# jasonyaw/CDAE

Hardware: AMD Instinct MI355X
Metric: users/sec (whole node) K=200 ML-10M-shape; Recall@10 parity (higher is better)
Workload: dtype f32

## Files before the change

cdae_amd/csrc/cdae_hip.hip:

```cpp
#include <hip/hip_runtime.h>

#include <cstring>

#include <rocprim/rocprim.hpp>

#include <algorithm>
#include <atomic>
#include <condition_variable>
#include <deque>
#include <mutex>
#include <thread>
#include <chrono>
#include <cmath>
#include <cstdarg>
#include <cstdlib>
#include <cstdio>
#include <cstring>
#include <numeric>
#include <string>
#include <vector>

#include "../../include/cdae_hip.h"
#include "cdae_internal.hpp"
#include "cdae_kernels.hpp"
#include "cdae_full_kernels.hpp"
#include "cdae_recommend_kernels.hpp"
#include "cdae_sort_kernels.hpp"
#include "cdae_mf_kernels.hpp"

#ifdef CDAE_DECODE_TIMING
#define CDAE_TOUCHED_ARG ((uint32_t*)nullptr)
#else
#define CDAE_TOUCHED_ARG h->d_touched
#endif

namespace {

thread_local std::string g_err;

int fail(const char* fmt, ...) {
  char buf[1024];
  va_list ap;
  va_start(ap, fmt);
  vsnprintf(buf, sizeof buf, fmt, ap);
  va_end(ap);
  g_err = buf;
  return 1;
}

#define HIPCHK(expr)                                                                           \
  do {                                                                                         \
    hipError_t e__ = (expr);                                                                   \
    if (e__ != hipSuccess)                                                                     \
      return fail("%s failed: %s (%s:%d)", #expr, hipGetErrorString(e__), __FILE__, __LINE__); \
  } while (0)

#define CHK(expr)            \
  do {                       \
    int rc__ = (expr);       \
    if (rc__) return rc__;   \
  } while (0)

#define DISPATCH_NI(ni, KERNEL, grid, block, shmem, stream, ...)                                  \
  do {                                                                                            \
    switch (ni) {                                                                                 \
      case 1: hipLaunchKernelGGL(KERNEL<1>, grid, block, shmem, stream, __VA_ARGS__); break;      \
      case 2: hipLaunchKernelGGL(KERNEL<2>, grid, block, shmem, stream, __VA_ARGS__); break;      \
      case 4: hipLaunchKernelGGL(KERNEL<4>, grid, block, shmem, stream, __VA_ARGS__); break;      \
      default: hipLaunchKernelGGL(KERNEL<8>, grid, block, shmem, stream, __VA_ARGS__); break;     \
    }                                                                                             \
  } while (0)

constexpr uint32_t MF_SEQ_USERS = 256;
constexpr uint32_t ENCODE_USERS_MAX = 768;
enum Family { F_SAMPLE = 0, F_SORT, F_ENCODE, F_DECODE, F_HIDDEN, F_INPUT, F_COUNT };

struct Span { int family; hipEvent_t a, b; };

}
// ... 1311 lines not shown
  CHK(dev_alloc(&h->d_shared, h->n_shared));
  HIPCHK(hipMemset(h->d_shared, 0, h->n_shared * sizeof(float)));
  const size_t WR = (size_t)h->wu_rows();
  h->cnt[CDAE_P_WU] = h->cnt[CDAE_P_WU_AG] = WR * h->Kp;
  CHK(dev_alloc(&h->d_Wu, WR * h->Kp));
  CHK(dev_alloc(&h->d_Wu_ag, WR * h->Kp));
  HIPCHK(hipMemset(h->d_Wu, 0, std::max<size_t>(WR * h->Kp, 1) * sizeof(float)));
  HIPCHK(hipMemset(h->d_Wu_ag, 0, std::max<size_t>(WR * h->Kp, 1) * sizeof(float)));
  if (h->cfg.linear_function) {
    h->cnt[CDAE_P_UU] = h->cnt[CDAE_P_UU_AG] = WR * h->Kp;
    CHK(dev_alloc(&h->d_Uu, WR * h->Kp));
    CHK(dev_alloc(&h->d_Uu_ag, WR * h->Kp));
  }

  const uint32_t B = (uint32_t)std::min<uint64_t>(h->B, U);
  uint64_t emax = 0;
  for (uint64_t s0 = 0; s0 < U; ++s0) {
    const uint64_t s1 = std::min<uint64_t>(U, s0 + B);
    emax = std::max<uint64_t>(emax, (uint64_t)(row_ptr[s1] - row_ptr[s0]));
  }
  h->ex_per_pos = h->mf == 2 ? 2u * h->hp.num_neg : 1u + h->hp.num_neg;
  h->Ecap = emax * h->ex_per_pos;
  h->h_grow_ptr.clear(); h->h_gunit_ptr.clear();
  if (h->shard_sampled()) {
    const int64_t* grp = h->g_row_ptr_src;
    const uint32_t* gcl = h->g_col_src;
    h->g_row_ptr_src = nullptr; h->g_col_src = nullptr;
    if (grp[0] != 0) return fail("whole-row row_ptr[0] must be 0");
    h->h_grow_ptr.assign(grp, grp + U + 1);
    uint64_t gmax = 0;
    for (uint64_t s0 = 0; s0 < U; ++s0) gmax = std::max<uint64_t>(gmax, (uint64_t)(grp[std::min<uint64_t>(U, s0 + B)] - grp[s0]));
    h->Ecap = gmax * h->ex_per_pos;
    const size_t gnnz = (size_t)grp[U];
    CHK(dev_alloc(&h->d_grow_ptr, U + 1)); CHK(dev_alloc(&h->d_gcol, gnnz));
    HIPCHK(hipMemcpy(h->d_grow_ptr, grp, (U + 1) * sizeof(int64_t), hipMemcpyHostToDevice));
    HIPCHK(hipMemcpy(h->d_gcol, gcl, gnnz * sizeof(uint32_t), hipMemcpyHostToDevice));
    h->h_gunit_ptr.assign(U + 1, 0u);
    for (uint64_t u = 0; u < U; ++u)
      h->h_gunit_ptr[u + 1] = h->h_gunit_ptr[u] + (uint32_t)((grp[u + 1] - grp[u] + h->hp.unit_pos - 1) / h->hp.unit_pos);
    CHK(dev_alloc(&h->d_gunit_ptr, U + 1));
    HIPCHK(hipMemcpy(h->d_gunit_ptr, h->h_gunit_ptr.data(), (U + 1) * sizeof(uint32_t), hipMemcpyHostToDevice));
    std::vector<uint32_t> guser(h->h_gunit_ptr[U]);
    for (uint64_t u = 0; u < U; ++u)
      for (uint32_t g = h->h_gunit_ptr[u]; g < h->h_gunit_ptr[u + 1]; ++g) guser[g] = (uint32_t)u;
    CHK(dev_alloc(&h->d_gunit_user, std::max<size_t>(guser.size(), 1)));
    HIPCHK(hipMemcpy(h->d_gunit_user, guser.data(), guser.size() * sizeof(uint32_t), hipMemcpyHostToDevice));
  }
  h->seq = 0; h->pre_n = 0;
  h->counting_sort = I <= cdae::TILE_SORT_MAX_ITEMS && DEV_ENV("CDAE_SORT_TILE") != nullptr;
  h->bucket_sort = false; h->bucket_ranges = 0; h->cell_units = 0;
  {
    const uint64_t BUCKET_MAX_EXAMPLES = h->cfg.full_output ? 100000 : 600000;
    const uint64_t keys = I + (h->shard_sampled() ? 1u : 0u);
    if (keys <= 65536 && !h->counting_sort && !h->mf_seq && h->Ecap <= BUCKET_MAX_EXAMPLES && h->Ecap > 0 && !DEV_ENV("CDAE_SORT_LIBRARY")) {
      const double b_share = (double)B / (double)U;
      const double draw_items = (double)(h->shard_sampled() ? h->I_global : I);
      const double whole_nnz = h->shard_sampled() ? (double)h->h_grow_ptr[U] : (double)nnz;
      const uint32_t negs = h->mf == 2 ? 2u * h->hp.num_neg - 0u : h->hp.num_neg;
      const double neg_per_item = b_share * whole_nnz * (double)negs / draw_items;
      std::vector<double> wgt(I);
      double total = 0.0;
      for (uint64_t i = 0; i < I; ++i) { wgt[i] = b_share * (double)pop[i] + neg_per_item; total += wgt[i]; }
      const double per_range = std::max(total / 256.0, std::min(2730.0, total / 8.0));
      std::vector<uint32_t> cut{0u};
      double acc = 0.0;
      for (uint64_t i = 0; i < I; ++i) {
        acc += wgt[i];
        if (i + 1 < I && (acc >= per_range || (i + 1) - cut.back() == cdae::BK_ITEMS)) { cut.push_back((uint32_t)(i + 1)); acc = 0.0; }
      }
      cut.push_back((uint32_t)I);
      if (cut.size() - 1 <= cdae::BK_MAX_RANGES) {
        h->bucket_sort = true;
        h->bucket_ranges = (uint32_t)cut.size() - 1;
        CHK(dev_alloc(&h->d_bucket_cut, cut.size()));
        HIPCHK(hipMemcpy(h->d_bucket_cut, cut.data(), cut.size() * sizeof(uint32_t), hipMemcpyHostToDevice));
        if (!h->mf && h->bucket_ranges <= cdae::BKC_MAX_RANGES && h->Ecap < (1ull << (32 - cdae::BKC_ITEM_BITS)) && !DEV_ENV("CDAE_SORT_SCAN")) {
          std::vector<uint16_t> rof(I);
          for (uint32_t r = 0; r + 1 < cut.size(); ++r)
            for (uint32_t i = cut[r]; i < cut[r + 1]; ++i) rof[i] = (uint16_t)r;
          CHK(dev_alloc(&h->d_range_of, (size_t)I));
          HIPCHK(hipMemcpy(h->d_range_of, rof.data(), I * sizeof(uint16_t), hipMemcpyHostToDevice));
        }
      }
    }
  }
  h->h_unit_ptr.assign(U + 1, 0u);
  for (uint64_t u = 0; u < U; ++u)
    h->h_unit_ptr[u + 1] = h->h_unit_ptr[u] + (uint32_t)((row_ptr[u + 1] - row_ptr[u] + h->hp.unit_pos - 1) / h->hp.unit_pos);
  h->unit_cap = 0;
  for (uint64_t s0 = 0; s0 < U; ++s0) {
    const uint64_t s1 = std::min<uint64_t>(U, s0 + B);
    h->unit_cap = std::max(h->unit_cap, h->h_unit_ptr[s1] - h->h_unit_ptr[s0]);
  }
  {
    std::vector<uint32_t> per(U);
    for (uint64_t u = 0; u < U; ++u) per[u] = h->h_unit_ptr[u + 1] - h->h_unit_ptr[u];
    std::partial_sort(per.begin(), per.begin() + B, per.end(), std::greater<uint32_t>());
    uint64_t top = 0;
    for (uint32_t i = 0; i < B; ++i) top += per[i];
    h->unit_cap = (uint32_t)std::max<uint64_t>(h->unit_cap, top);
  }
  if (h->shard_sampled())
    for (uint64_t s0 = 0; s0 < U; ++s0)
      h->unit_cap = std::max(h->unit_cap, h->h_gunit_ptr[std::min<uint64_t>(U, s0 + B)] - h->h_gunit_ptr[s0]);
  CHK(dev_alloc(&h->d_unit_ptr, U + 1));
  HIPCHK(hipMemcpy(h->d_unit_ptr, h->h_unit_ptr.data(), (U + 1) * sizeof(uint32_t), hipMemcpyHostToDevice));
  {
    std::vector<uint32_t> unit_user(h->h_unit_ptr[U]);
    for (uint64_t u = 0; u < U; ++u)
      for (uint32_t g = h->h_unit_ptr[u]; g < h->h_unit_ptr[u + 1]; ++g) unit_user[g] = (uint32_t)u;
    CHK(dev_alloc(&h->d_unit_user, std::max<size_t>(unit_user.size(), 1)));
    HIPCHK(hipMemcpy(h->d_unit_user, unit_user.data(), unit_user.size() * sizeof(uint32_t), hipMemcpyHostToDevice));
  }
  CHK(dev_alloc(&h->d_Hpart, (size_t)h->unit_cap * h->Kp));
  CHK(dev_alloc(&h->d_uptr_tmp, (size_t)B + 1));
  {
    const uint32_t one_unit[2] = {0u, 1u};
    HIPCHK(hipMemcpy(h->d_uptr_tmp, one_unit, sizeof one_unit, hipMemcpyHostToDevice));
  }
  if ((uint64_t)B * h->Kp * sizeof(float) > 0x7FFFFFFFull)
    return fail("batch_users %u x row stride %u floats exceeds the 2 GiB the batch's Z may occupy; lower batch_users", B, h->Kp);
  if (h->Ecap > 0xFFFFFFF0ull) return fail("batch of %u users holds %llu examples (> 2^32); lower batch_users", B, (unsigned long long)h->Ecap);
  for (auto& b : h->ex) {
// ... 1410 lines not shown
```

cdae_amd/csrc/cdae_kernels.hpp:

```cpp
#pragma once
#include <type_traits>

#include <hip/hip_runtime.h>
#include <stdint.h>

#include "../../include/cdae_rng.h"
#include "cdae_exchange_algebra.h"

namespace cdae {

constexpr int WAVE = 64;
constexpr uint32_t SLOT_MASK = 0x0FFFFFFFu;
constexpr uint32_t DUP_PREV_BIT = 1u << 28;
constexpr uint32_t DUP_NEXT_BIT = 1u << 29;
constexpr uint32_t DUP_NONE = 0xFFFFFFFFu;
constexpr uint32_t DUP_STRIPES = 64;
constexpr uint32_t TARGET_BIT = 1u << 30;
constexpr uint32_t INPUT_BIT = 1u << 31;

constexpr uint32_t LATE_MAX = 64;
struct DecodeLate {
  float* Ghot;
  uint32_t* hotdup;
  uint32_t late_rows;
// ... 1393 lines not shown
      if (dup) { const uint32_t k = len + (uint32_t)__popcll(dmask & below); lrow[k] = cur.di[h2] | DUP_ROW; lg[k] = 1.f; }
      if (mine) { const uint32_t k = len + n_d + (uint32_t)__popcll(mask & below); lrow[k] = cur.item[h2]; lg[k] = cur.g[h2]; }
      len += n_d + n_r;
    }
    __builtin_amdgcn_fence(__ATOMIC_RELEASE, "wavefront");
    __builtin_amdgcn_wave_barrier();
    const bool last = c0 + 2 * WAVE >= n_ex;
    while (len - head >= (uint32_t)TRIP) trip((uint32_t)TRIP);
    if (last || len + 4u * WAVE > GCAP) {
      if (len > head) trip(len - head);
      head = 0; len = 0;
      __builtin_amdgcn_wave_barrier();
    }
    cur = nxt;
  }
  if (lo >= hp.K) {
#pragma unroll
    for (int i = 0; i < NI; ++i) acc[i] = 0.f;
  }
  vstore<NI>(ga.HGpart + ((size_t)part * ga.n_units + unit) * hp.Kp + lo, acc);
  trace_end(hp, 5, unit * 8u + part, t0, n_ex);
}

template <int NI>
__global__ void __launch_bounds__(256)
hidden_gather_kernel(HyperParams hp, const int64_t* __restrict__ row_ptr, const uint32_t* __restrict__ uptr,
                     uint32_t n_units, uint64_t u0, uint32_t nb, const uint32_t* __restrict__ ex_item,
                     const float* __restrict__ G, const float* __restrict__ D0,
                     float* __restrict__ HGpart ,
                     uint32_t explicit_examples ,
                     const uint32_t* __restrict__ dup_of_ex, const float* __restrict__ dup_corr,
                     const uint32_t* __restrict__ unit_user,
                     const uint32_t* __restrict__ late_bits = nullptr ,
                     uint32_t late_words = 0) {
  __shared__ uint32_t gl_row[4][GATHER_CAP];
  __shared__ float gl_g[4][GATHER_CAP];
  __shared__ uint32_t lbits[LATE_BITS_WORDS];
  stage_late_bits(lbits, late_bits, late_words);
  const uint32_t part = blockIdx.x & 7u;
  const uint32_t unit = (blockIdx.x >> 3) * (blockDim.x / WAVE) + threadIdx.x / WAVE;
  if (unit >= n_units) return;
  const GatherArgs ga{row_ptr, uptr, n_units, u0, nb, ex_item, G, D0, HGpart, explicit_examples, dup_of_ex, dup_corr, unit_user,
                      late_bits, late_words, nullptr};
  hidden_gather_role<NI, false>(hp, ga, part, unit, gl_row[threadIdx.x / WAVE], gl_g[threadIdx.x / WAVE], late_bits ? lbits : nullptr);
}

struct FusedGeom {
  uint32_t hot_wgs;
  uint32_t decode_wgs;
  const uint32_t* cold_map;
};
constexpr uint32_t FUSED_LDS_WORDS = 4u * 2u * GATHER_CAP + LATE_BITS_WORDS;
static_assert(4u * ROWS16_LDS_WORDS <= FUSED_LDS_WORDS, "row roles' LDS");
static_assert(3u * (FUSED_LDS_WORDS + 8u) * 4u + 90376u <= 160u * 1024u, "three workgroups of this launch + one of bucket_sort_kernel per CU");
#ifndef CDAE_FUSED_WAVES_PER_SIMD
#define CDAE_FUSED_WAVES_PER_SIMD 3
#endif
template <int NV, int NT, int LOSS, bool ADAGRAD>
__global__ void __launch_bounds__(256, CDAE_FUSED_WAVES_PER_SIMD)
decode_gather_kernel(HyperParams hp, uint32_t hot_rows, FusedGeom geo, DecodeLate late, GatherArgs ga, CDAE_DECODE_PARAMS) {
  constexpr int CH = NT == 0 ? NV : NV + 1;
  constexpr int NI = CH <= 1 ? 1 : (CH <= 2 ? 2 : 4);
  __shared__ uint32_t fused_lds[FUSED_LDS_WORDS + 8u];
  const uint32_t wg = blockIdx.x;
  const uint32_t wid = __builtin_amdgcn_readfirstlane(threadIdx.x / WAVE);
  if (wg < geo.hot_wgs) {
    const uint32_t row = wg * 4u + wid;
    if (row < hot_rows && !CDAE_SKIP_ROLE(hp, 4u)) {
      const unsigned long long t0 = trace_begin(hp);
      __builtin_amdgcn_s_setprio(CDAE_HOT_PRIO);
      decode_row64<NI, LOSS, ADAGRAD, false, true>(hp, row, reinterpret_cast<float*>(fused_lds + wid * ROWS16_LDS_WORDS), ROW64_PARK_WORDS, late,
                                                   CDAE_DECODE_PASS);
      __builtin_amdgcn_s_setprio(0);
      trace_end(hp, 3, row, t0, hp.trace ? hw_place() : 0u);
    }
  } else if (wg < geo.decode_wgs) {
    if (CDAE_SKIP_ROLE(hp, 8u)) return;
    uint32_t* const claim = fused_lds + FUSED_LDS_WORDS;
    if (threadIdx.x < 4) claim[threadIdx.x] = 0u;
    __syncthreads();
    const uint32_t simd = (__builtin_amdgcn_s_getreg((1 << 11) | (4 << 6) | 4) ) & 3u;
    if (threadIdx.x % WAVE == 0) atomicCAS(&claim[simd], 0u, 1u + wid);
    __syncthreads();
    const uint32_t cs[4] = {claim[0], claim[1], claim[2], claim[3]};
    int mine = -1;
#pragma unroll
    for (int q = 0; q < 4; ++q) if (cs[q] == 1u + wid) mine = q;
    if (mine < 0) {
      uint32_t before = 0, cnt = 0;
#pragma unroll
      for (int q = 0; q < 4; ++q) if (cs[q] && cs[q] - 1u < wid) ++before;
      const uint32_t j = wid - before;
#pragma unroll
      for (int q = 0; q < 4; ++q) if (!cs[q]) { if (cnt == j) mine = q; ++cnt; }
    }
    const uint32_t g = geo.cold_map[wg * 4u + (uint32_t)mine];
    if (g == 0xFFFFFFFFu) return;
    const unsigned long long t0 = trace_begin(hp);
    decode_rows16<NV, NT, LOSS, ADAGRAD, true>(hp, hot_rows + g * 4u, fused_lds + wid * ROWS16_LDS_WORDS, CDAE_DECODE_PASS);
    trace_end(hp, 4, hot_rows / 4u + g, t0, hp.trace ? hw_place() : 0u);
  } else {
    uint32_t* const lbits = fused_lds + 4u * 2u * GATHER_CAP;
    stage_late_bits(lbits, ga.late_bits, ga.late_words);
    const uint32_t gw = wg - geo.decode_wgs;
    const uint32_t part = gw & 7u, unit = (gw >> 3) * 4u + wid;
    if (unit >= ga.n_units) return;
    hidden_gather_role<NI, true>(hp, ga, part, unit, fused_lds + wid * 2u * GATHER_CAP,
// ... 718 lines not shown
```

cdae_amd/csrc/cdae_sort_kernels.hpp:

```cpp
#pragma once
#include <hip/hip_runtime.h>
#include <stdint.h>

#include "cdae_kernels.hpp"

namespace cdae {

#ifndef CDAE_SEGSORT_THREADS
#define CDAE_SEGSORT_THREADS 256
#endif
constexpr uint32_t SEGSORT_THREADS = CDAE_SEGSORT_THREADS;
#ifndef CDAE_SEGSORT_ITEMS
#define CDAE_SEGSORT_ITEMS 8
#endif
constexpr uint32_t SEGSORT_ITEMS = CDAE_SEGSORT_ITEMS;
#ifndef CDAE_SEGSORT_WINDOW
#define CDAE_SEGSORT_WINDOW 3072
#endif
constexpr uint32_t SEGSORT_WINDOW = CDAE_SEGSORT_WINDOW;

constexpr uint32_t TILE_SORT_MAX_ITEMS = 32768;
#ifndef CDAE_TILE_EX
#define CDAE_TILE_EX 4096
#endif
// ... 143 lines not shown
        const uint64_t v = raw[q];
        uint32_t r[8] = {0, 0, 0, 0, 0, 0, 0, 0};
        uint32_t j = a;
        for (; j + 8 <= b; j += 8) {
#pragma unroll
          for (int t = 0; t < 8; ++t) r[t] += raw[j + t] < v ? 1u : 0u;
        }
        for (; j < b; ++j) r[0] += raw[j] < v ? 1u : 0u;
        rank = ((r[0] + r[1]) + (r[2] + r[3])) + ((r[4] + r[5]) + (r[6] + r[7]));
        srt[a + rank] = v;
      } else {
        const uint64_t v = bucketed_val[p0 + q];
        for (uint32_t j = a; j < b; ++j) rank += bucketed_val[p0 + j] < v ? 1u : 0u;
        sorted_val[p0 + a + rank] = v;
      }
    }
    __syncthreads();
    uint32_t my_dups = 0;
    for (uint32_t q = threadIdx.x; q < n; q += blockDim.x) {
      const uint32_t k = item_of(k0, p0 + q);
      const uint32_t a = item_off[k] - p0, b = item_off[k + 1] - p0;
      uint64_t v = in_lds ? srt[q] : sorted_val[p0 + q];
      const uint32_t slot = (uint32_t)v & SLOT_MASK;
      uint32_t flags = 0;
      if (q > a && ((uint32_t)(in_lds ? srt[q - 1] : sorted_val[p0 + q - 1]) & SLOT_MASK) == slot) flags |= DUP_PREV_BIT;
      if (q + 1 < b && ((uint32_t)(in_lds ? srt[q + 1] : sorted_val[p0 + q + 1]) & SLOT_MASK) == slot) flags |= DUP_NEXT_BIT;
      if (in_lds || flags) sorted_val[p0 + q] = v | flags;
      if (flags & DUP_PREV_BIT) ++my_dups;
    }
    uint32_t off = my_dups ? atomicAdd(&blk_count, my_dups) : 0u;
    __syncthreads();
    if (threadIdx.x == 0) { blk_base = blk_count ? atomicAdd(dup_count + blockIdx.x % stripes, blk_count) : 0u; blk_count = 0u; }
    __syncthreads();
    if (my_dups) {
      off += blk_base;
      const uint32_t stripe_cap = dup_cap / stripes, stripe0 = (blockIdx.x % stripes) * stripe_cap;
      for (uint32_t q = threadIdx.x; q < n; q += blockDim.x) {
        const uint64_t v = sorted_val[p0 + q];
        if (!((uint32_t)v & DUP_PREV_BIT)) continue;
        const uint32_t idx = off < stripe_cap ? stripe0 + off : DUP_NONE;
        ++off;
        dup_of_pos[p0 + q] = idx;
        dup_of_ex[(uint32_t)(v >> 32)] = idx;
      }
    }
    __syncthreads();
    k0 = k1;
  }
}

constexpr uint32_t BK_THREADS = 512;
constexpr uint32_t BK_WINDOW = 4096;
constexpr uint32_t BK_ITEMS = 2048;
constexpr uint32_t BK_WAVE_LIST = BK_WINDOW / (BK_THREADS / 64);
constexpr uint32_t BK_SPIN_CAP = 1u << 21;
constexpr uint32_t BK_MAX_RANGES = 1024;
constexpr uint32_t BK_CELL_UNITS_MAX = 16384;
constexpr size_t BK_LDS_BYTES = (size_t)BK_WINDOW * 8 * 2 + (size_t)BK_WINDOW * 2 + (size_t)(BK_ITEMS + 1) * 4 * 2 + 64 * 4;
static_assert(BK_ITEMS <= 4 * BK_THREADS && BK_ITEMS <= (1u << BKC_ITEM_BITS), "bk_block_scan takes 4 counters per thread; a cell entry holds the item in BKC_ITEM_BITS bits");

__device__ __forceinline__ void bk_block_scan(uint32_t* v, uint32_t n, uint32_t* wave_tot) {
  const uint32_t t = threadIdx.x, lane = t % WAVE, wid = t / WAVE;
  uint32_t c[4], sum = 0;
#pragma unroll
  for (uint32_t j = 0; j < 4; ++j) { c[j] = 4u * t + j < n ? v[4u * t + j] : 0u; sum += c[j]; }
  uint32_t incl = sum;
#pragma unroll
  for (int off = 1; off < WAVE; off <<= 1) {
    const uint32_t o = __shfl_up(incl, off, WAVE);
    if ((int)lane >= off) incl += o;
  }
  if (lane == WAVE - 1) wave_tot[wid] = incl;
  __syncthreads();
  uint32_t before = 0;
  for (uint32_t w = 0; w < wid; ++w) before += wave_tot[w];
  uint32_t run = before + incl - sum;
#pragma unroll
  for (uint32_t j = 0; j < 4; ++j) { if (4u * t + j < n) v[4u * t + j] = run; run += c[j]; }
  if (t == BK_THREADS - 1) v[n] = run;
  __syncthreads();
}

constexpr uint32_t BK_UNROLL = 4;
template <typename F>
__device__ __forceinline__ void bk_scan_keys(const uint16_t* __restrict__ keys, uint32_t n_ex, F&& f) {
  const uint32_t n8 = n_ex & ~7u;
  constexpr uint32_t ROUND = BK_THREADS * 8u * BK_UNROLL;
  uint4 q[BK_UNROLL], nx[BK_UNROLL];
  auto request = [&](uint4 (&dst)[BK_UNROLL], uint32_t r0) {
#pragma unroll
    for (uint32_t u = 0; u < BK_UNROLL; ++u) {
      const uint32_t e0 = r0 + (u * BK_THREADS + threadIdx.x) * 8u;
      dst[u] = e0 < n8 ? *reinterpret_cast<const uint4*>(keys + e0) : make_uint4(0xFFFFFFFFu, 0xFFFFFFFFu, 0xFFFFFFFFu, 0xFFFFFFFFu);
    }
  };
  request(q, 0u);
  for (uint32_t r0 = 0; r0 < n8; r0 += ROUND) {
    const bool more = r0 + ROUND < n8;
    if (more) request(nx, r0 + ROUND);
#pragma unroll
    for (uint32_t u = 0; u < BK_UNROLL; ++u) {
      const uint32_t e0 = r0 + (u * BK_THREADS + threadIdx.x) * 8u;
      if (r0 + u * BK_THREADS * 8u >= n8) break;
      const bool valid = e0 < n8;
      const uint32_t w[4] = {q[u].x, q[u].y, q[u].z, q[u].w};
#pragma unroll
      for (uint32_t j = 0; j < 4; ++j) { f(e0 + 2u * j, w[j] & 0xFFFFu, valid); f(e0 + 2u * j + 1u, w[j] >> 16, valid); }
    }
    if (more) {
#pragma unroll
      for (uint32_t u = 0; u < BK_UNROLL; ++u) q[u] = nx[u];
    }
  }
  if (n_ex != n8 && threadIdx.x < WAVE) {
    const bool valid = threadIdx.x < n_ex - n8;
    f(n8 + threadIdx.x, valid ? (uint32_t)keys[n8 + threadIdx.x] : 0u, valid);
  }
}

__global__ void __launch_bounds__(BK_THREADS)
bucket_sort_kernel(const uint16_t* __restrict__ keys, const uint64_t* __restrict__ ex_val, uint32_t n_ex,
                   const uint32_t* __restrict__ range_cut , uint32_t* __restrict__ wg_state ,
                   const uint32_t* __restrict__ cells , uint32_t cell_units,
                   const uint32_t* __restrict__ cell_flag , uint32_t cell_tag,
                   uint32_t* __restrict__ seg_begin, uint32_t* __restrict__ seg_end, const uint32_t* __restrict__ rank_of,
                   uint32_t* __restrict__ segr_begin, uint32_t* __restrict__ segr_end, uint64_t* __restrict__ sorted_val,
                   uint64_t* __restrict__ scratch_val ,
                   uint32_t* __restrict__ dup_count, uint32_t dup_cap, uint32_t* __restrict__ dup_of_pos,
                   uint32_t* __restrict__ dup_of_ex , uint32_t stripes,
                   uint32_t* __restrict__ err ) {
#ifdef CDAE_PREP_SETPRIO
  __builtin_amdgcn_s_setprio(CDAE_PREP_SETPRIO);
#endif
  extern __shared__ __attribute__((aligned(16))) unsigned char bk_lds[];
  uint64_t* raw = reinterpret_cast<uint64_t*>(bk_lds);
  uint64_t* srt = raw + BK_WINDOW;
  uint32_t* off = reinterpret_cast<uint32_t*>(srt + BK_WINDOW);
  uint32_t* cur = off + BK_ITEMS + 1;
  uint32_t* misc = cur + BK_ITEMS + 1;
  uint16_t* raw_item = reinterpret_cast<uint16_t*>(misc + 64);
  const uint32_t t = threadIdx.x, w = blockIdx.x, lane = t % WAVE;
  const uint32_t lo = range_cut[w], n_it = range_cut[w + 1] - lo;
  for (uint32_t i = t; i <= n_it; i += BK_THREADS) off[i] = 0u;
  if (t == 0) { misc[16] = 0u; misc[17] = 0u; misc[19] = 0u; }
  __syncthreads();

  bool listed = false;
  bool scanned = false;
  if (cells && cell_units <= BK_CELL_UNITS_MAX && *cell_flag != cell_tag) {
    uint16_t* wcnt = reinterpret_cast<uint16_t*>(raw);
    uint32_t* lst = reinterpret_cast<uint32_t*>(srt);
    uint16_t* tk = reinterpret_cast<uint16_t*>(lst + BK_WINDOW);
    const uint32_t* mine = cells + (size_t)w * cell_units * BKC_SLOTS;
    const uint32_t per = (cell_units + BK_THREADS - 1) / BK_THREADS, u0 = min(cell_units, t * per), u1 = min(cell_units, u0 + per);
    uint32_t sum = 0;
    for (uint32_t u = u0; u < u1; ++u) { const uint32_t c = mine[(size_t)u * BKC_SLOTS]; wcnt[u] = (uint16_t)c; sum += c; }
    uint32_t incl = sum;
#pragma unroll
    for (int o = 1; o < WAVE; o <<= 1) {
      const uint32_t v = __shfl_up(incl, o, WAVE);
      if ((int)lane >= o) incl += v;
    }
    if (lane == WAVE - 1) misc[t / WAVE] = incl;
    __syncthreads();
    uint32_t pos = incl - sum, total = 0;
    for (uint32_t v = 0; v < BK_THREADS / WAVE; ++v) { if (v < t / WAVE) pos += misc[v]; total += misc[v]; }
    __syncthreads();
    if (total <= BK_WINDOW) {
      for (uint32_t u = u0; u < u1; ++u) {
        const uint32_t c = wcnt[u];
        for (uint32_t j = 0; j < c; ++j) lst[pos + j] = mine[(size_t)u * BKC_SLOTS + 1u + j];
        pos += c;
      }
      __syncthreads();
      for (uint32_t i = t; i < total; i += BK_THREADS) tk[i] = (uint16_t)atomicAdd(&off[lst[i] & BKC_ITEM_MASK], 1u);
      __syncthreads();
      bk_block_scan(off, n_it, misc);
      for (uint32_t i = t; i < total; i += BK_THREADS) {
        const uint32_t ent = lst[i], d = ent & BKC_ITEM_MASK, p = off[d] + tk[i];
        raw[p] = ex_val[ent >> BKC_ITEM_BITS];
        raw_item[p] = (uint16_t)d;
      }
      listed = true; scanned = true;
    } else {
      for (uint32_t i = t; i <= n_it; i += BK_THREADS) off[i] = 0u;
      __syncthreads();
    }
  }

  uint64_t* const wave_list = srt + (t / WAVE) * BK_WAVE_LIST;
  uint32_t wave_n = 0;
  if (!scanned) {
    bk_scan_keys(keys, n_ex, [&](uint32_t e, uint32_t k, bool valid) {
      const uint32_t d = k - lo;
      const bool mine = valid && d < n_it;
      const uint64_t m = __ballot(mine);
      if (m == 0ull) return;
      if (mine) {
        const uint32_t ticket = atomicAdd(&off[d], 1u);
        const uint32_t slot = wave_n + __builtin_amdgcn_mbcnt_hi((uint32_t)(m >> 32), __builtin_amdgcn_mbcnt_lo((uint32_t)m, 0u));
        if (slot < BK_WAVE_LIST) wave_list[slot] = ((uint64_t)e << 32) | (uint64_t)(d << 16) | (uint64_t)(ticket & 0xFFFFu);
      }
      wave_n += (uint32_t)__popcll(m);
    });
    if (wave_n > BK_WAVE_LIST && lane == 0) misc[19] = 1u;
    __syncthreads();
    bk_block_scan(off, n_it, misc);
  }

  if (t == 0) __hip_atomic_store(&wg_state[w], off[n_it] + 1u, __ATOMIC_RELEASE, __HIP_MEMORY_SCOPE_AGENT);
  for (uint32_t r = t; r < w; r += BK_THREADS) {
    uint32_t v, spin = 0;
    while ((v = __hip_atomic_load(&wg_state[r], __ATOMIC_ACQUIRE, __HIP_MEMORY_SCOPE_AGENT)) == 0u) {
      if (++spin > BK_SPIN_CAP) { v = 1u; __hip_atomic_store(err, 2u, __ATOMIC_RELAXED, __HIP_MEMORY_SCOPE_SYSTEM); break; }
      __builtin_amdgcn_s_sleep(1);
    }
    atomicAdd(&misc[16], v - 1u);
  }
  __syncthreads();
  const uint32_t base = misc[16];
  for (uint32_t i = t; i < n_it; i += BK_THREADS) {
    const uint32_t c = off[i + 1] - off[i], b = c ? base + off[i] : 0u, e = c ? base + off[i + 1] : 0u;
    seg_begin[lo + i] = b; seg_end[lo + i] = e;
    if (rank_of) { const uint32_t r = rank_of[lo + i]; segr_begin[r] = b; segr_end[r] = e; }
  }
  const bool wave_listed = !listed && misc[19] == 0u && off[n_it] <= BK_WINDOW;

  uint32_t ia = 0;
  while (ia < n_it) {
    uint32_t ib = ia + 1;
    {
      uint32_t l = ia + 1, h = n_it;
      while (l < h) { const uint32_t mid = (l + h + 1) >> 1; if (off[mid] - off[ia] <= BK_WINDOW) l = mid; else h = mid - 1; }
      ib = l;
    }
    const uint32_t g0 = off[ia], n = off[ib] - g0;
    const bool in_lds = n <= BK_WINDOW;
    if (n == 0) { ia = ib; continue; }
    if (listed) {
    } else if (wave_listed) {
      for (uint32_t i = lane; i < wave_n; i += WAVE) {
        const uint64_t rec = wave_list[i];
        const uint32_t d = (uint32_t)(rec >> 16) & 0xFFFFu, p = off[d] + ((uint32_t)rec & 0xFFFFu);
        raw[p] = ex_val[(uint32_t)(rec >> 32)];
        raw_item[p] = (uint16_t)d;
      }
    } else {
      for (uint32_t i = ia + t; i < ib; i += BK_THREADS) cur[i] = off[i] - g0;
      __syncthreads();
      bk_scan_keys(keys, n_ex, [&](uint32_t e, uint32_t k, bool valid) {
        const uint32_t d = k - lo;
        if (valid && d - ia < ib - ia) {
          const uint32_t p = atomicAdd(&cur[d], 1u);
          const uint64_t v = ex_val[e];
          if (in_lds) { raw[p] = v; raw_item[p] = (uint16_t)d; } else scratch_val[base + g0 + p] = v;
        }
      });
    }
    __threadfence_block();
    __syncthreads();
    for (uint32_t q = t; q < n; q += BK_THREADS) {
      if (in_lds) {
        const uint32_t d = raw_item[q], a = off[d] - g0, b = off[d + 1] - g0;
        const uint64_t v = raw[q];
        uint32_t r[8] = {0, 0, 0, 0, 0, 0, 0, 0};
        uint32_t j = a;
        for (; j + 8 <= b; j += 8) {
#pragma unroll
          for (int u = 0; u < 8; ++u) r[u] += raw[j + u] < v ? 1u : 0u;
        }
        for (; j < b; ++j) r[0] += raw[j] < v ? 1u : 0u;
        srt[a + ((r[0] + r[1]) + (r[2] + r[3])) + ((r[4] + r[5]) + (r[6] + r[7]))] = v;
      } else {
        const uint64_t v = scratch_val[base + g0 + q];
        uint32_t rank = 0;
        for (uint32_t j = 0; j < n; ++j) rank += scratch_val[base + g0 + j] < v ? 1u : 0u;
        sorted_val[base + g0 + rank] = v;
      }
    }
    __threadfence_block();
    __syncthreads();
    uint32_t my_dups = 0;
    for (uint32_t q = t; q < n; q += BK_THREADS) {
      uint32_t a = 0, b = n;
      if (in_lds) {
        uint32_t l = ia, h = ib - 1;
        while (l < h) { const uint32_t mid = (l + h + 1) >> 1; if (off[mid] - g0 <= q) l = mid; else h = mid - 1; }
        a = off[l] - g0; b = off[l + 1] - g0;
      }
      const uint64_t v = in_lds ? srt[q] : sorted_val[base + g0 + q];
      const uint32_t slot = (uint32_t)v & SLOT_MASK;
      uint32_t flags = 0;
      if (q > a && ((uint32_t)(in_lds ? srt[q - 1] : sorted_val[base + g0 + q - 1]) & SLOT_MASK) == slot) flags |= DUP_PREV_BIT;
      if (q + 1 < b && ((uint32_t)(in_lds ? srt[q + 1] : sorted_val[base + g0 + q + 1]) & SLOT_MASK) == slot) flags |= DUP_NEXT_BIT;
      if (in_lds || flags) sorted_val[base + g0 + q] = v | flags;
      if (flags & DUP_PREV_BIT) ++my_dups;
    }
    uint32_t o = my_dups ? atomicAdd(&misc[17], my_dups) : 0u;
    __syncthreads();
    if (t == 0) { misc[18] = misc[17] ? atomicAdd(dup_count + w % stripes, misc[17]) : 0u; misc[17] = 0u; }
    __syncthreads();
    if (my_dups) {
      o += misc[18];
      const uint32_t stripe_cap = dup_cap / stripes, stripe0 = (w % stripes) * stripe_cap;
      for (uint32_t q = t; q < n; q += BK_THREADS) {
        const uint64_t v = sorted_val[base + g0 + q];
        if (!((uint32_t)v & DUP_PREV_BIT)) continue;
        const uint32_t idx = o < stripe_cap ? stripe0 + o : DUP_NONE;
        ++o;
        dup_of_pos[base + g0 + q] = idx;
        dup_of_ex[(uint32_t)(v >> 32)] = idx;
      }
    }
    __syncthreads();
    ia = ib;
  }
}

}
```

Before: 2.904 million.

## Shrink bucket sort LDS to 32-bit keys and vectorise cell gather

Result: no change. 2.902 million (-0.1%).

```diff
diff --git a/cdae_amd/csrc/cdae_hip.hip b/cdae_amd/csrc/cdae_hip.hip
--- a/cdae_amd/csrc/cdae_hip.hip
+++ b/cdae_amd/csrc/cdae_hip.hip
@@ -25,6 +25,7 @@
 #include "cdae_kernels.hpp"
 #include "cdae_full_kernels.hpp"
 #include "cdae_recommend_kernels.hpp"
+#include "cdae_range_cut.h"
 #include "cdae_sort_kernels.hpp"
 #include "cdae_mf_kernels.hpp"
 
@@ -1442,23 +1443,13 @@
   {
     const uint64_t BUCKET_MAX_EXAMPLES = h->cfg.full_output ? 100000 : 600000;
     const uint64_t keys = I + (h->shard_sampled() ? 1u : 0u);
-    if (keys <= 65536 && !h->counting_sort && !h->mf_seq && h->Ecap <= BUCKET_MAX_EXAMPLES && h->Ecap > 0 && !DEV_ENV("CDAE_SORT_LIBRARY")) {
+    if (keys <= 65536 && !h->counting_sort && !h->mf_seq && h->Ecap <= BUCKET_MAX_EXAMPLES && h->Ecap < cdae::BK_MAX_EXAMPLES && h->Ecap > 0 && !DEV_ENV("CDAE_SORT_LIBRARY")) {
       const double b_share = (double)B / (double)U;
       const double draw_items = (double)(h->shard_sampled() ? h->I_global : I);
       const double whole_nnz = h->shard_sampled() ? (double)h->h_grow_ptr[U] : (double)nnz;
       const uint32_t negs = h->mf == 2 ? 2u * h->hp.num_neg - 0u : h->hp.num_neg;
       const double neg_per_item = b_share * whole_nnz * (double)negs / draw_items;
-      std::vector<double> wgt(I);
-      double total = 0.0;
-      for (uint64_t i = 0; i < I; ++i) { wgt[i] = b_share * (double)pop[i] + neg_per_item; total += wgt[i]; }
-      const double per_range = std::max(total / 256.0, std::min(2730.0, total / 8.0));
-      std::vector<uint32_t> cut{0u};
-      double acc = 0.0;
-      for (uint64_t i = 0; i < I; ++i) {
-        acc += wgt[i];
-        if (i + 1 < I && (acc >= per_range || (i + 1) - cut.back() == cdae::BK_ITEMS)) { cut.push_back((uint32_t)(i + 1)); acc = 0.0; }
-      }
-      cut.push_back((uint32_t)I);
+      const std::vector<uint32_t> cut = cdae::range_cut(pop.data(), I, b_share, neg_per_item, cdae::BK_RANGE_TARGET, cdae::BK_ITEMS);
       if (cut.size() - 1 <= cdae::BK_MAX_RANGES) {
         h->bucket_sort = true;
         h->bucket_ranges = (uint32_t)cut.size() - 1;
diff --git a/cdae_amd/csrc/cdae_kernels.hpp b/cdae_amd/csrc/cdae_kernels.hpp
--- a/cdae_amd/csrc/cdae_kernels.hpp
+++ b/cdae_amd/csrc/cdae_kernels.hpp
@@ -1469,7 +1469,8 @@
 };
 constexpr uint32_t FUSED_LDS_WORDS = 4u * 2u * GATHER_CAP + LATE_BITS_WORDS;
 static_assert(4u * ROWS16_LDS_WORDS <= FUSED_LDS_WORDS, "row roles' LDS");
-static_assert(3u * (FUSED_LDS_WORDS + 8u) * 4u + 90376u <= 160u * 1024u, "three workgroups of this launch + one of bucket_sort_kernel per CU");
+constexpr uint32_t BK_LDS_BOUND = 45u * 1024u;
+static_assert(3u * (FUSED_LDS_WORDS + 8u) * 4u + 2u * BK_LDS_BOUND <= 160u * 1024u, "three workgroups of this launch + two of bucket_sort_kernel per CU");
 #ifndef CDAE_FUSED_WAVES_PER_SIMD
 #define CDAE_FUSED_WAVES_PER_SIMD 3
 #endif
diff --git a/cdae_amd/csrc/cdae_range_cut.h b/cdae_amd/csrc/cdae_range_cut.h
--- /dev/null
+++ b/cdae_amd/csrc/cdae_range_cut.h
@@ -0,0 +1,30 @@
+#pragma once
+#include <stdint.h>
+
+#include <algorithm>
+#include <vector>
+
+namespace cdae {
+
+inline double range_cut_weight(uint64_t pop_i, double batch_share, double neg_per_item) { return batch_share * (double)pop_i + neg_per_item; }
+
+inline double range_cut_target(double total_weight, uint32_t target_examples) {
+  return std::max(total_weight / 256.0, std::min((double)target_examples, total_weight / 8.0));
+}
+
+inline std::vector<uint32_t> range_cut(const uint64_t* pop, uint64_t num_items, double batch_share, double neg_per_item,
+                                       uint32_t target_examples, uint32_t max_items) {
+  double total = 0.0;
+  for (uint64_t i = 0; i < num_items; ++i) total += range_cut_weight(pop[i], batch_share, neg_per_item);
+  const double per_range = range_cut_target(total, target_examples);
+  std::vector<uint32_t> cut{0u};
+  double acc = 0.0;
+  for (uint64_t i = 0; i < num_items; ++i) {
+    acc += range_cut_weight(pop[i], batch_share, neg_per_item);
+    if (i + 1 < num_items && (acc >= per_range || (i + 1) - cut.back() == max_items)) { cut.push_back((uint32_t)(i + 1)); acc = 0.0; }
+  }
+  cut.push_back((uint32_t)num_items);
+  return cut;
+}
+
+}
diff --git a/cdae_amd/csrc/cdae_sort_kernels.hpp b/cdae_amd/csrc/cdae_sort_kernels.hpp
--- a/cdae_amd/csrc/cdae_sort_kernels.hpp
+++ b/cdae_amd/csrc/cdae_sort_kernels.hpp
@@ -219,12 +219,19 @@
 constexpr uint32_t BK_THREADS = 512;
 constexpr uint32_t BK_WINDOW = 4096;
 constexpr uint32_t BK_ITEMS = 2048;
+constexpr uint32_t BK_RANGE_TARGET = 2730;
+constexpr uint32_t BK_PER_THREAD = BK_WINDOW / BK_THREADS;
 constexpr uint32_t BK_WAVE_LIST = BK_WINDOW / (BK_THREADS / 64);
 constexpr uint32_t BK_SPIN_CAP = 1u << 21;
 constexpr uint32_t BK_MAX_RANGES = 1024;
 constexpr uint32_t BK_CELL_UNITS_MAX = 16384;
-constexpr size_t BK_LDS_BYTES = (size_t)BK_WINDOW * 8 * 2 + (size_t)BK_WINDOW * 2 + (size_t)(BK_ITEMS + 1) * 4 * 2 + 64 * 4;
+constexpr uint32_t BK_MAX_EXAMPLES = 1u << (32 - BKC_ITEM_BITS);
+constexpr uint32_t BK_CELL_LOADS = 4;
+constexpr size_t BK_LDS_BYTES = (size_t)BK_WINDOW * 4 * 2 + (size_t)(BK_ITEMS + 1) * 4 + 64 * 4;
 static_assert(BK_ITEMS <= 4 * BK_THREADS && BK_ITEMS <= (1u << BKC_ITEM_BITS), "bk_block_scan takes 4 counters per thread; a cell entry holds the item in BKC_ITEM_BITS bits");
+static_assert(BK_ITEMS + 1 <= BK_WINDOW, "the group cursors of the scan fallback live in the sorted-entries array");
+static_assert(BK_LDS_BYTES <= BK_LDS_BOUND, "two workgroups per CU beside three of the decode launch (cdae_kernels.hpp)");
+static_assert(BKC_SLOTS == 32 && BK_THREADS % 8 == 0, "the gather takes a cell with eight 16-byte loads");
 
 __device__ __forceinline__ void bk_block_scan(uint32_t* v, uint32_t n, uint32_t* wave_tot) {
   const uint32_t t = threadIdx.x, lane = t % WAVE, wid = t / WAVE;
@@ -245,6 +252,18 @@
 #pragma unroll
   for (uint32_t j = 0; j < 4; ++j) { if (4u * t + j < n) v[4u * t + j] = run; run += c[j]; }
   if (t == BK_THREADS - 1) v[n] = run;
+  __syncthreads();
+}
+
+__device__ __forceinline__ void bk_shift_back(uint32_t* v, uint32_t n) {
+  const uint32_t t = threadIdx.x;
+  uint32_t c[4];
+  __syncthreads();
+#pragma unroll
+  for (uint32_t j = 0; j < 4; ++j) { const uint32_t i = 4u * t + j; c[j] = i > 0u && i < n ? v[i - 1u] : 0u; }
+  __syncthreads();
+#pragma unroll
+  for (uint32_t j = 0; j < 4; ++j) { const uint32_t i = 4u * t + j; if (i < n) v[i] = c[j]; }
   __syncthreads();
 }
 
@@ -286,7 +305,7 @@
 }
 
 __global__ void __launch_bounds__(BK_THREADS)
-bucket_sort_kernel(const uint16_t* __restrict__ keys, const uint64_t* __restrict__ ex_val, uint32_t n_ex,
+bucket_sort_kernel(const uint16_t* __restrict__ keys, const uint64_t* __restrict__ ex_val, uint32_t n_ex ,
                    const uint32_t* __restrict__ range_cut , uint32_t* __restrict__ wg_state ,
                    const uint32_t* __restrict__ cells , uint32_t cell_units,
                    const uint32_t* __restrict__ cell_flag , uint32_t cell_tag,
@@ -300,62 +319,76 @@
   __builtin_amdgcn_s_setprio(CDAE_PREP_SETPRIO);
 #endif
   extern __shared__ __attribute__((aligned(16))) unsigned char bk_lds[];
-  uint64_t* raw = reinterpret_cast<uint64_t*>(bk_lds);
-  uint64_t* srt = raw + BK_WINDOW;
-  uint32_t* off = reinterpret_cast<uint32_t*>(srt + BK_WINDOW);
-  uint32_t* cur = off + BK_ITEMS + 1;
-  uint32_t* misc = cur + BK_ITEMS + 1;
-  uint16_t* raw_item = reinterpret_cast<uint16_t*>(misc + 64);
+  uint32_t* raw = reinterpret_cast<uint32_t*>(bk_lds);
+  uint32_t* srt = raw + BK_WINDOW;
+  uint32_t* off = srt + BK_WINDOW;
+  uint32_t* misc = off + BK_ITEMS + 1;
+  uint32_t* cur = srt;
   const uint32_t t = threadIdx.x, w = blockIdx.x, lane = t % WAVE;
   const uint32_t lo = range_cut[w], n_it = range_cut[w + 1] - lo;
   for (uint32_t i = t; i <= n_it; i += BK_THREADS) off[i] = 0u;
-  if (t == 0) { misc[16] = 0u; misc[17] = 0u; misc[19] = 0u; }
+  if (t == 0) { misc[16] = 0u; misc[17] = 0u; misc[19] = 0u; misc[20] = 0u; }
   __syncthreads();
 
   bool listed = false;
   bool scanned = false;
-  if (cells && cell_units <= BK_CELL_UNITS_MAX && *cell_flag != cell_tag) {
-    uint16_t* wcnt = reinterpret_cast<uint16_t*>(raw);
-    uint32_t* lst = reinterpret_cast<uint32_t*>(srt);
-    uint16_t* tk = reinterpret_cast<uint16_t*>(lst + BK_WINDOW);
+  if (cells && *cell_flag != cell_tag) {
     const uint32_t* mine = cells + (size_t)w * cell_units * BKC_SLOTS;
-    const uint32_t per = (cell_units + BK_THREADS - 1) / BK_THREADS, u0 = min(cell_units, t * per), u1 = min(cell_units, u0 + per);
-    uint32_t sum = 0;
-    for (uint32_t u = u0; u < u1; ++u) { const uint32_t c = mine[(size_t)u * BKC_SLOTS]; wcnt[u] = (uint16_t)c; sum += c; }
-    uint32_t incl = sum;
-#pragma unroll
-    for (int o = 1; o < WAVE; o <<= 1) {
-      const uint32_t v = __shfl_up(incl, o, WAVE);
-      if ((int)lane >= o) incl += v;
-    }
-    if (lane == WAVE - 1) misc[t / WAVE] = incl;
-    __syncthreads();
-    uint32_t pos = incl - sum, total = 0;
-    for (uint32_t v = 0; v < BK_THREADS / WAVE; ++v) { if (v < t / WAVE) pos += misc[v]; total += misc[v]; }
-    __syncthreads();
+    const uint32_t sub = t % 8u, cell0 = t / 8u, head = lane & ~7u;
+    constexpr uint32_t ROUND = (BK_THREADS / 8u) * BK_CELL_LOADS;
+    for (uint32_t u0 = 0; u0 < cell_units; u0 += ROUND) {
+      uint4 cw[BK_CELL_LOADS];
+#pragma unroll
+      for (uint32_t k = 0; k < BK_CELL_LOADS; ++k) {
+        const uint32_t u = u0 + k * (BK_THREADS / 8u) + cell0;
+        cw[k] = u < cell_units ? *reinterpret_cast<const uint4*>(mine + (size_t)u * BKC_SLOTS + 4u * sub) : make_uint4(0u, 0u, 0u, 0u);
+      }
+#pragma unroll
+      for (uint32_t k = 0; k < BK_CELL_LOADS; ++k) {
+        const uint32_t c = min((uint32_t)__shfl((int)cw[k].x, (int)head, WAVE), BKC_SLOTS - 1u);
+        const uint32_t ent[4] = {cw[k].x, cw[k].y, cw[k].z, cw[k].w};
+        bool ok[4];
+        uint64_t m[4];
+        uint32_t found = 0;
+#pragma unroll
+        for (uint32_t j = 0; j < 4; ++j) {
+          const uint32_t wi = 4u * sub + j;
+          ok[j] = wi >= 1u && wi <= c && (ent[j] & BKC_ITEM_MASK) < n_it;
+          m[j] = __ballot(ok[j]);
+          found += (uint32_t)__popcll(m[j]);
+        }
+        if (found == 0u) continue;
+        uint32_t slot0 = 0;
+        if (lane == 0) slot0 = atomicAdd(&misc[20], found);
+        slot0 = __builtin_amdgcn_readfirstlane(slot0);
+#pragma unroll
+        for (uint32_t j = 0; j < 4; ++j) {
+          if (ok[j]) {
+            const uint32_t slot = slot0 + __builtin_amdgcn_mbcnt_hi((uint32_t)(m[j] >> 32), __builtin_amdgcn_mbcnt_lo((uint32_t)m[j], 0u));
+            if (slot < BK_WINDOW) { srt[slot] = ent[j]; atomicAdd(&off[ent[j] & BKC_ITEM_MASK], 1u); }
+          }
+          slot0 += (uint32_t)__popcll(m[j]);
+        }
+      }
+    }
+    __syncthreads();
+    const uint32_t total = misc[20];
     if (total <= BK_WINDOW) {
-      for (uint32_t u = u0; u < u1; ++u) {
-        const uint32_t c = wcnt[u];
-        for (uint32_t j = 0; j < c; ++j) lst[pos + j] = mine[(size_t)u * BKC_SLOTS + 1u + j];
-        pos += c;
-      }
-      __syncthreads();
-      for (uint32_t i = t; i < total; i += BK_THREADS) tk[i] = (uint16_t)atomicAdd(&off[lst[i] & BKC_ITEM_MASK], 1u);
-      __syncthreads();
       bk_block_scan(off, n_it, misc);
       for (uint32_t i = t; i < total; i += BK_THREADS) {
-        const uint32_t ent = lst[i], d = ent & BKC_ITEM_MASK, p = off[d] + tk[i];
-        raw[p] = ex_val[ent >> BKC_ITEM_BITS];
-        raw_item[p] = (uint16_t)d;
-      }
+        const uint32_t e = srt[i];
+        raw[atomicAdd(&off[e & BKC_ITEM_MASK], 1u)] = e;
+      }
+      bk_shift_back(off, n_it);
       listed = true; scanned = true;
     } else {
+      __syncthreads();
       for (uint32_t i = t; i <= n_it; i += BK_THREADS) off[i] = 0u;
       __syncthreads();
     }
   }
 
-  uint64_t* const wave_list = srt + (t / WAVE) * BK_WAVE_LIST;
+  uint32_t* const wave_list = srt + (t / WAVE) * BK_WAVE_LIST;
   uint32_t wave_n = 0;
   if (!scanned) {
     bk_scan_keys(keys, n_ex, [&](uint32_t e, uint32_t k, bool valid) {
@@ -364,9 +397,9 @@
       const uint64_t m = __ballot(mine);
       if (m == 0ull) return;
       if (mine) {
-        const uint32_t ticket = atomicAdd(&off[d], 1u);
+        atomicAdd(&off[d], 1u);
         const uint32_t slot = wave_n + __builtin_amdgcn_mbcnt_hi((uint32_t)(m >> 32), __builtin_amdgcn_mbcnt_lo((uint32_t)m, 0u));
-        if (slot < BK_WAVE_LIST) wave_list[slot] = ((uint64_t)e << 32) | (uint64_t)(d << 16) | (uint64_t)(ticket & 0xFFFFu);
+        if (slot < BK_WAVE_LIST) wave_list[slot] = (e << BKC_ITEM_BITS) | d;
       }
       wave_n += (uint32_t)__popcll(m);
     });
@@ -406,12 +439,12 @@
     if (n == 0) { ia = ib; continue; }
     if (listed) {
     } else if (wave_listed) {
+      __syncthreads();
       for (uint32_t i = lane; i < wave_n; i += WAVE) {
-        const uint64_t rec = wave_list[i];
-        const uint32_t d = (uint32_t)(rec >> 16) & 0xFFFFu, p = off[d] + ((uint32_t)rec & 0xFFFFu);
-        raw[p] = ex_val[(uint32_t)(rec >> 32)];
-        raw_item[p] = (uint16_t)d;
-      }
+        const uint32_t e = wave_list[i];
+        raw[atomicAdd(&off[e & BKC_ITEM_MASK], 1u)] = e;
+      }
+      bk_shift_back(off, n_it);
     } else {
       for (uint32_t i = ia + t; i < ib; i += BK_THREADS) cur[i] = off[i] - g0;
       __syncthreads();
@@ -419,17 +452,17 @@
         const uint32_t d = k - lo;
         if (valid && d - ia < ib - ia) {
           const uint32_t p = atomicAdd(&cur[d], 1u);
-          const uint64_t v = ex_val[e];
-          if (in_lds) { raw[p] = v; raw_item[p] = (uint16_t)d; } else scratch_val[base + g0 + p] = v;
+          if (in_lds) raw[p] = (e << BKC_ITEM_BITS) | d; else scratch_val[base + g0 + p] = ex_val[e];
         }
       });
     }
     __threadfence_block();
     __syncthreads();
-    for (uint32_t q = t; q < n; q += BK_THREADS) {
-      if (in_lds) {
-        const uint32_t d = raw_item[q], a = off[d] - g0, b = off[d + 1] - g0;
-        const uint64_t v = raw[q];
+    uint32_t my_dups = 0, dup_bits = 0;
+    uint64_t word[BK_PER_THREAD];
+    if (in_lds) {
+      for (uint32_t q = t; q < n; q += BK_THREADS) {
+        const uint32_t v = raw[q], d = v & BKC_ITEM_MASK, a = off[d] - g0, b = off[d + 1] - g0;
         uint32_t r[8] = {0, 0, 0, 0, 0, 0, 0, 0};
         uint32_t j = a;
         for (; j + 8 <= b; j += 8) {
@@ -438,30 +471,50 @@
         }
         for (; j < b; ++j) r[0] += raw[j] < v ? 1u : 0u;
         srt[a + ((r[0] + r[1]) + (r[2] + r[3])) + ((r[4] + r[5]) + (r[6] + r[7]))] = v;
-      } else {
+      }
+      __syncthreads();
+#pragma unroll
+      for (uint32_t k = 0; k < BK_PER_THREAD; ++k) {
+        const uint32_t q = k * BK_THREADS + t;
+        word[k] = q < n ? ex_val[srt[q] >> BKC_ITEM_BITS] : 0ull;
+      }
+#pragma unroll
+      for (uint32_t k = 0; k < BK_PER_THREAD; ++k) {
+        const uint32_t q = k * BK_THREADS + t;
+        if (q < n) raw[q] = (uint32_t)word[k];
+      }
+      __syncthreads();
+#pragma unroll
+      for (uint32_t k = 0; k < BK_PER_THREAD; ++k) {
+        const uint32_t q = k * BK_THREADS + t;
+        if (q < n) {
+          const uint32_t d = srt[q] & BKC_ITEM_MASK, a = off[d] - g0, b = off[d + 1] - g0;
+          const uint32_t slot = (uint32_t)word[k] & SLOT_MASK;
+          uint32_t flags = 0;
+          if (q > a && (raw[q - 1] & SLOT_MASK) == slot) flags |= DUP_PREV_BIT;
+          if (q + 1 < b && (raw[q + 1] & SLOT_MASK) == slot) flags |= DUP_NEXT_BIT;
+          sorted_val[base + g0 + q] = word[k] | flags;
+          if (flags & DUP_PREV_BIT) { ++my_dups; dup_bits |= 1u << k; }
+        }
+      }
+    } else {
+      for (uint32_t q = t; q < n; q += BK_THREADS) {
         const uint64_t v = scratch_val[base + g0 + q];
         uint32_t rank = 0;
         for (uint32_t j = 0; j < n; ++j) rank += scratch_val[base + g0 + j] < v ? 1u : 0u;
         sorted_val[base + g0 + rank] = v;
       }
-    }
-    __threadfence_block();
-    __syncthreads();
-    uint32_t my_dups = 0;
-    for (uint32_t q = t; q < n; q += BK_THREADS) {
-      uint32_t a = 0, b = n;
-      if (in_lds) {
-        uint32_t l = ia, h = ib - 1;
-        while (l < h) { const uint32_t mid = (l + h + 1) >> 1; if (off[mid] - g0 <= q) l = mid; else h = mid - 1; }
-        a = off[l] - g0; b = off[l + 1] - g0;
-      }
-      const uint64_t v = in_lds ? srt[q] : sorted_val[base + g0 + q];
-      const uint32_t slot = (uint32_t)v & SLOT_MASK;
-      uint32_t flags = 0;
-      if (q > a && ((uint32_t)(in_lds ? srt[q - 1] : sorted_val[base + g0 + q - 1]) & SLOT_MASK) == slot) flags |= DUP_PREV_BIT;
-      if (q + 1 < b && ((uint32_t)(in_lds ? srt[q + 1] : sorted_val[base + g0 + q + 1]) & SLOT_MASK) == slot) flags |= DUP_NEXT_BIT;
-      if (in_lds || flags) sorted_val[base + g0 + q] = v | flags;
-      if (flags & DUP_PREV_BIT) ++my_dups;
+      __threadfence_block();
+      __syncthreads();
+      for (uint32_t q = t; q < n; q += BK_THREADS) {
+        const uint64_t v = sorted_val[base + g0 + q];
+        const uint32_t slot = (uint32_t)v & SLOT_MASK;
+        uint32_t flags = 0;
+        if (q > 0 && ((uint32_t)sorted_val[base + g0 + q - 1] & SLOT_MASK) == slot) flags |= DUP_PREV_BIT;
+        if (q + 1 < n && ((uint32_t)sorted_val[base + g0 + q + 1] & SLOT_MASK) == slot) flags |= DUP_NEXT_BIT;
+        if (flags) sorted_val[base + g0 + q] = v | flags;
+        if (flags & DUP_PREV_BIT) ++my_dups;
+      }
     }
     uint32_t o = my_dups ? atomicAdd(&misc[17], my_dups) : 0u;
     __syncthreads();
@@ -470,13 +523,24 @@
     if (my_dups) {
       o += misc[18];
       const uint32_t stripe_cap = dup_cap / stripes, stripe0 = (w % stripes) * stripe_cap;
-      for (uint32_t q = t; q < n; q += BK_THREADS) {
-        const uint64_t v = sorted_val[base + g0 + q];
-        if (!((uint32_t)v & DUP_PREV_BIT)) continue;
-        const uint32_t idx = o < stripe_cap ? stripe0 + o : DUP_NONE;
-        ++o;
-        dup_of_pos[base + g0 + q] = idx;
-        dup_of_ex[(uint32_t)(v >> 32)] = idx;
+      if (in_lds) {
+#pragma unroll
+        for (uint32_t k = 0; k < BK_PER_THREAD; ++k) {
+          if (!(dup_bits >> k & 1u)) continue;
+          const uint32_t idx = o < stripe_cap ? stripe0 + o : DUP_NONE;
+          ++o;
+          dup_of_pos[base + g0 + k * BK_THREADS + t] = idx;
+          dup_of_ex[(uint32_t)(word[k] >> 32)] = idx;
+        }
+      } else {
+        for (uint32_t q = t; q < n; q += BK_THREADS) {
+          const uint64_t v = sorted_val[base + g0 + q];
+          if (!((uint32_t)v & DUP_PREV_BIT)) continue;
+          const uint32_t idx = o < stripe_cap ? stripe0 + o : DUP_NONE;
+          ++o;
+          dup_of_pos[base + g0 + q] = idx;
+          dup_of_ex[(uint32_t)(v >> 32)] = idx;
+        }
       }
     }
     __syncthreads();
```
